# ZikangYuan/sr_livo

Hardware: AMD Instinct MI355X
Metric: sweeps/s (full ESIKF solve of a 64k-pt Livox sweep vs 1M-pt voxel map) (higher is better)
Workload: dtype f64; 1 GPU; HEADLINE: stream of 4 distinct 65536-keypoint livox sweeps (own poses and priors), 978481-pt voxel map (1000000 target), max_num_residuals=2147483647, r=1, K=20; one full ESIKF solve per sweep, every sweep crosses PCIe once (uploaded on the copy stream during the solve before it: resident in HBM when its solve starts); sweeps drawn with seeds 20251309 + 100 j, keeping those that take sweep 0's 2 E; parallelism=single GPU

## Files before the change

include/srlivo_hip_debug.h:

```cpp
#ifndef SRLIVO_HIP_DEBUG_H
#define SRLIVO_HIP_DEBUG_H

#include "srlivo_hip.h"

#ifdef __cplusplus
extern "C" {
#endif

int srl_debug_set_select_mode(srl_ctx *ctx, int select_mode);

int srl_debug_radix_sort_pairs(srl_ctx *ctx, const uint32_t *keys, int n, int bits, uint32_t *keys_sorted, uint32_t *positions_sorted);

int srl_debug_color_map_rebuilds(srl_ctx *ctx, int32_t *voxel_table, int32_t *grid_table);

int srl_debug_set_frame_order_mode(srl_ctx *ctx, int mode);
int srl_debug_frame_order_used(srl_ctx *ctx, int *used);

int srl_debug_set_gather_counts(srl_ctx *ctx, int nranks, int rank, const int64_t *counts);

int srl_debug_set_ablate(srl_ctx *ctx, int bits);
int srl_debug_set_fused_reduce(srl_ctx *ctx, int enable);
int srl_debug_set_bound_culling(srl_ctx *ctx, int enable);
int srl_debug_set_pose_box(srl_ctx *ctx, int kind);
int srl_debug_set_arm_linger(srl_ctx *ctx, double host_linger_us, double kernel_linger_us);
int srl_debug_pass_stamps(srl_ctx *ctx, int enable, long long *gpu_out, long long *host_out);
int srl_debug_frame_timing(srl_ctx *ctx, int enable, double out16[16]);
int srl_debug_set_frame_epoch(srl_ctx *ctx, int frames_to_wrap);
int srl_debug_set_launch_shape(srl_ctx *ctx, int keypoints_per_wave, int waves_per_workgroup);
int srl_debug_set_search_select_mode(srl_ctx *ctx, int select_mode);
int srl_debug_heap_topk(const double *distances, int n, int K, int32_t *out_index);
int srl_debug_device_sqrt(srl_ctx *ctx, const double *in, int n, double *out);
int srl_debug_block_times(srl_ctx *ctx, double *out, int max_blocks, int *nblocks);

#ifdef __cplusplus
}
#endif
#endif
```

sr_livo_amd/capi.py:

```python
import ctypes as C
import os
import re

import numpy as np

_HERE = os.path.dirname(os.path.abspath(__file__))
LIB_PATH = os.environ.get("SRL_LIB_PATH") or os.path.join(_HERE, "libsrlivo_hip.so")
INCLUDE_DIR = os.path.join(os.path.dirname(_HERE), "include")

SRL_OK = 0
SRL_ERR_NO_DEVICE = -1
SRL_ERR_UNSUPPORTED = -4
SRL_ERR_COMM = -7
SRL_ERR_NAN_PLANARITY = -8
SRL_ERR_NOT_ENOUGH_RESIDUALS = -9
SRL_COMM_ID_BYTES = 128


SRL_PEER_HANDLE_BYTES = 64


class SrlError(RuntimeError):
    def __init__(self, status, what, detail=""):
        self.status = status
# ... 112 lines not shown
        "srl_color_map_insert": ([p, p, C.c_int, C.c_double, C.c_double, p, p, C.c_int, p, C.c_int, C.POINTER(ColorTotals)], C.c_int),
        "srl_color_map_size": ([p, C.POINTER(C.c_int64), C.POINTER(C.c_int32), C.POINTER(C.c_int64), C.POINTER(C.c_int64)], C.c_int),
        "srl_color_map_download": ([p, p, p, p, C.c_int, p, p, C.c_int64], C.c_int),
        "srl_color_registered_download": ([p, C.c_int64, C.c_int, p], C.c_int),
        "srl_debug_color_map_rebuilds": ([p, C.POINTER(C.c_int32), C.POINTER(C.c_int32)], C.c_int),
        "srl_sweep_upload": ([p, p, C.c_int], C.c_int),
        "srl_sweep_shard": ([p, C.POINTER(C.c_int), C.POINTER(C.c_int), C.POINTER(C.c_int)], C.c_int),
        "srl_sweep_prefetch": ([p, p, C.c_int], C.c_int),
        "srl_sweep_swap": ([p], C.c_int),
        "srl_sweep_wait": ([p], C.c_int),
        "srl_thread_pin_to_gpu_numa": ([p, C.POINTER(C.c_int)], C.c_int),
        "srl_pinned_alloc": ([C.c_size_t, C.POINTER(p)], C.c_int),
        "srl_pinned_free": ([p], C.c_int),
        "srl_host_register": ([p, C.c_size_t], C.c_int),
        "srl_host_unregister": ([p], C.c_int),
        "srl_comm_backend_info": ([C.c_char_p, C.c_int, C.POINTER(C.c_int), C.POINTER(C.c_int)], C.c_int),
        "srl_build_residuals": ([p, C.POINTER(Frame), C.POINTER(IcpOpts), C.POINTER(NormalEq)], C.c_int),
        "srl_build_residuals_overlap": ([p, C.POINTER(Frame), C.POINTER(IcpOpts), C.POINTER(NormalEq), p, p], C.c_int),
        "srl_set_taps": ([p, C.c_int], C.c_int),
        "srl_fetch_neighbors": ([p, p, p, p], C.c_int),
        "srl_fetch_residuals": ([p, p, p, p, p, p, p], C.c_int),
        "srl_search_neighbors": ([p, p, C.c_int, C.c_int, C.c_double, C.c_int, C.c_int, p, p, p], C.c_int),
        "srl_transform_points": ([p, p, C.c_int, dp, dp, dp, dp, p], C.c_int),
        "srl_frame_upload": ([p, p, C.c_int], C.c_int),
        "srl_frame_undistort": ([p, p, p, p, C.c_int, p, C.c_int, C.c_double, C.c_int, dp, dp, p, p], C.c_int),
        "srl_frame_take": ([p, p, C.c_int], C.c_int),
        "srl_frame_subsample": ([p, p, C.c_int, C.c_double, C.POINTER(C.c_int)], C.c_int),
        "srl_frame_take_subsampled": ([p, p, C.c_int, p, p, p], C.c_int),
        "srl_frame_size": ([p, C.POINTER(C.c_int)], C.c_int),
        "srl_frame_select_keypoints": ([p, dp, dp, dp, dp, C.c_double, p, C.POINTER(C.c_int)], C.c_int),
        "srl_frame_commit_report": ([p, dp, dp, dp, dp, C.c_double, C.c_int, C.c_double, C.c_int, p, p, p, C.POINTER(C.c_int),
                                     C.POINTER(C.c_int)], C.c_int),
        "srl_frame_commit": ([p, dp, dp, dp, dp, C.c_double, C.c_int, C.c_double, C.c_int, p, C.POINTER(C.c_int)], C.c_int),
        "srl_comm_unique_id": ([p], C.c_int),
        "srl_comm_init_rank": ([p, C.c_int, C.c_int, p], C.c_int),
        "srl_comm_destroy": ([p], C.c_int),
        "srl_comm_set_library": ([C.c_char_p], C.c_int),
        "srl_comm_suspend": ([p, C.c_int], C.c_int),
        "srl_comm_info": ([p, C.POINTER(C.c_int), C.POINTER(C.c_int), C.POINTER(C.c_int), C.POINTER(C.c_int), C.POINTER(C.c_int64)], C.c_int),
        "srl_comm_set_host_callbacks": ([p, C.c_int, C.c_int, ALLREDUCE_FN, ALLGATHER_FN, p], C.c_int),
        "srl_debug_set_gather_counts": ([p, C.c_int, C.c_int, C.POINTER(C.c_int64)], C.c_int),
        "srl_peer_export": ([p, p, C.POINTER(p)], C.c_int),
        "srl_peer_attach": ([p, C.c_int, C.c_int, p, C.POINTER(p)], C.c_int),
        "srl_peer_set_deadline_ms": ([p, C.c_int], C.c_int),
        "srl_peer_stats": ([p, C.POINTER(C.c_int64), C.POINTER(C.c_int)], C.c_int),
        "srl_peer_detach": ([p], C.c_int),
        "srl_shard_range": ([C.c_int, C.c_int, C.c_int, C.POINTER(C.c_int), C.POINTER(C.c_int)], None),
        "srl_shard_budget": ([C.c_int, C.POINTER(C.c_int64), C.c_int, C.c_int, C.POINTER(C.c_int64), C.POINTER(C.c_int)], None),
        "srl_get_timing": ([p, C.POINTER(Timing)], C.c_int),
        "srl_debug_block_times": ([p, p, C.c_int, C.POINTER(C.c_int)], C.c_int),
        "srl_debug_set_ablate": ([p, C.c_int], C.c_int),
        "srl_debug_set_fused_reduce": ([p, C.c_int], C.c_int),
        "srl_debug_set_bound_culling": ([p, C.c_int], C.c_int),
        "srl_debug_set_pose_box": ([p, C.c_int], C.c_int),
        "srl_debug_set_arm_linger": ([p, C.c_double, C.c_double], C.c_int),
        "srl_debug_pass_stamps": ([p, C.c_int, p, p], C.c_int),
        "srl_debug_frame_timing": ([p, C.c_int, p], C.c_int),
        "srl_debug_set_frame_epoch": ([p, C.c_int], C.c_int),
        "srl_set_armed_launch": ([p, C.c_int], C.c_int),
        "srl_disarm": ([p], C.c_int),
        "srl_solve_end": ([p], C.c_int),
        "srl_get_arm_stats": ([p, C.POINTER(C.c_uint64)], C.c_int),
        "srl_debug_set_launch_shape": ([p, C.c_int, C.c_int], C.c_int),
        "srl_debug_set_search_select_mode": ([p, C.c_int], C.c_int),
        "srl_debug_set_select_mode": ([p, C.c_int], C.c_int),
        "srl_debug_set_frame_order_mode": ([p, C.c_int], C.c_int),
        "srl_debug_radix_sort_pairs": ([p, p, C.c_int, C.c_int, p, p], C.c_int),
        "srl_debug_frame_order_used": ([p, C.POINTER(C.c_int)], C.c_int),
        "srl_debug_heap_topk": ([p, C.c_int, C.c_int, p], C.c_int),
        "srl_debug_device_sqrt": ([p, p, C.c_int, p], C.c_int),
        "srl_set_profiling": ([p, C.c_int], C.c_int),
        "srl_set_profiling_period": ([p, C.c_int], C.c_int),
        "srl_timing_mark": ([p], C.c_int),
        "srl_lio_create": ([C.c_int, C.POINTER(p)], C.c_int),
        "srl_lio_destroy": ([p], C.c_int),
        "srl_lio_ctx": ([p], p),
        "srl_lio_last_error": ([p], C.c_char_p),
        "srl_lio_set_extrinsics": ([p, dp, dp], C.c_int),
        "srl_lio_set_laser_point_cov": ([p, C.c_double], C.c_int),
        "srl_lio_last_solve_launches": ([p, C.POINTER(C.c_int)], C.c_int),
        "srl_lio_eskf_get_state": ([p, dp], C.c_int),
        "srl_lio_eskf_set_state": ([p, dp], C.c_int),
        "srl_lio_eskf_get_cov": ([p, dp], C.c_int),
        "srl_lio_eskf_set_cov": ([p, dp], C.c_int),
        "srl_lio_eskf_set_noise": ([p, C.c_double, C.c_double, C.c_double, C.c_double], C.c_int),
        "srl_lio_eskf_init_imu": ([p, dp, dp], C.c_int),
        "srl_lio_eskf_scale_init_cov": ([p], C.c_int),
        "srl_lio_eskf_predict": ([p, C.c_double, dp, dp], C.c_int),
        "srl_lio_eskf_observe": ([p, dp], C.c_int),
        "srl_lio_add_points_to_map": ([p, p, C.c_int, C.c_double, C.c_int, C.c_double, C.c_int], C.c_int),
        "srl_lio_map_size": ([p, C.POINTER(C.c_int64)], C.c_int),
        "srl_lio_remove_points_far_from_location": ([p, dp, C.c_double], C.c_int),
        "srl_lio_set_collect_points_world": ([p, C.c_int], C.c_int),
        "srl_lio_points_world": ([p, p, C.c_int, C.POINTER(C.c_int)], C.c_int),
        "srl_lio_set_device_subsample": ([p, C.c_int], C.c_int),
        "srl_lio_set_color_map_options": ([p, C.POINTER(ColorOpts)], C.c_int),
        "srl_lio_set_color_times": ([p, C.c_double, C.c_double, C.c_int], C.c_int),
        "srl_lio_add_points_to_map_at": ([p, p, C.c_int, C.c_double, C.c_int, C.c_double, C.c_int, C.c_double, C.c_int], C.c_int),
        "srl_lio_color_visited": ([p, C.c_int, p, C.c_int, C.POINTER(C.c_int), C.POINTER(C.c_int)], C.c_int),
        "srl_lio_color_stored": ([p, p, C.c_int, C.POINTER(C.c_int)], C.c_int),
        "srl_lio_probe_checksum_of_committed_frame": ([p, C.c_int, C.c_double, C.POINTER(C.c_uint64), C.POINTER(C.c_int32)], C.c_int),
        "srl_lio_resident_sweep": ([p, p, C.c_int], C.c_int),
        "srl_lio_prefetch_sweep": ([p, p, C.c_int], C.c_int),
        "srl_lio_swap_sweep": ([p], C.c_int),
        "srl_lio_prefetch_sweep_during_solve": ([p, p, C.c_int], C.c_int),
        "srl_lio_update_iekf": ([p, C.POINTER(IcpOpts), p, C.c_int, dp, dp, C.c_int, p, C.c_int,
# ... 344 lines not shown
            self._chk(self.lib.srl_debug_set_select_mode(self.h, mode), "srl_debug_set_select_mode")
            self._select_mode = mode

    def build_residuals(self, frame, opts, allow=(SRL_ERR_NAN_PLANARITY,)):
        self._select(opts)
        out = NormalEq()
        rc = self._chk(self.lib.srl_build_residuals(self.h, C.byref(frame), C.byref(opts), C.byref(out)), "srl_build_residuals", ok=allow)
        return out, rc

    def build_residuals_overlap(self, frame, opts, fn, allow=(SRL_ERR_NAN_PLANARITY,)):
        self._select(opts)
        out = NormalEq()
        cb = C.CFUNCTYPE(None, C.c_void_p)(lambda _u: fn())
        rc = self._chk(self.lib.srl_build_residuals_overlap(self.h, C.byref(frame), C.byref(opts), C.byref(out), cb, None),
                       "srl_build_residuals_overlap", ok=allow)
        return out, rc

    def pin_thread_to_gpu_numa(self):
        node = C.c_int(-1)
        rc = self.lib.srl_thread_pin_to_gpu_numa(self.h, C.byref(node))
        return node.value if rc == 0 else None

    def fetch_neighbors(self, K=20):
        _, n, _ = self.sweep_shard()
        ids = np.empty((n, K), dtype=np.int32)
        status = np.empty(n, dtype=np.uint8)
        ncand = np.empty(n, dtype=np.int32)
        self._chk(self.lib.srl_fetch_neighbors(self.h, _ptr(ids), _ptr(status), _ptr(ncand)), "srl_fetch_neighbors")
        return ids, status, ncand

    def fetch_residuals(self):
        _, n, _ = self.sweep_shard()
        normal = np.empty((n, 3)); a2d = np.empty(n); w = np.empty(n); off = np.empty(n); d = np.empty(n); J = np.empty((n, 6))
        self._chk(self.lib.srl_fetch_residuals(self.h, _ptr(normal), _ptr(a2d), _ptr(w), _ptr(off), _ptr(d), _ptr(J)), "srl_fetch_residuals")
        return dict(normal=normal, a2D=a2d, weight=w, norm_offset=off, distance=d, jacobian=J)

    def search_neighbors(self, world_xyz, nb=1, size=1.0, K=20, thr=1):
        q = _f64(world_xyz, (-1, 3))
        ids = np.empty((len(q), K), dtype=np.int32)
        xyz = np.empty((len(q), K, 3), dtype=np.float32)
        nf = np.empty(len(q), dtype=np.int32)
        self._chk(self.lib.srl_search_neighbors(self.h, _ptr(q), len(q), nb, size, K, thr, _ptr(ids), _ptr(xyz), _ptr(nf)), "srl_search_neighbors")
        return ids, xyz, nf

    def set_launch_shape(self, kpw, wpb):
        self._chk(self.lib.srl_debug_set_launch_shape(self.h, int(kpw), int(wpb)), "srl_debug_set_launch_shape")

    def set_fused_reduce(self, on):
        self._chk(self.lib.srl_debug_set_fused_reduce(self.h, 1 if on else 0), "srl_debug_set_fused_reduce")

    def set_bound_culling(self, on):
        self._chk(self.lib.srl_debug_set_bound_culling(self.h, 1 if on else 0), "srl_debug_set_bound_culling")

    def set_search_select_mode(self, mode):
        self._chk(self.lib.srl_debug_set_search_select_mode(self.h, int(mode)), "srl_debug_set_search_select_mode")

    def set_armed_launch(self, on):
        mode = int(on) if on in (0, 1, 2) and not isinstance(on, bool) else (1 if on else 0)
        self._chk(self.lib.srl_set_armed_launch(self.h, mode), "srl_set_armed_launch")

    def solve_end(self):
        self._chk(self.lib.srl_solve_end(self.h), "srl_solve_end")

    def disarm(self):
        self._chk(self.lib.srl_disarm(self.h), "srl_disarm")

    def arm_stats(self):
        out = (C.c_uint64 * 4)()
        self._chk(self.lib.srl_get_arm_stats(self.h, out), "srl_get_arm_stats")
        return dict(zip(("armed", "fired", "cancelled", "expired"), (int(v) for v in out)))

    def set_pose_box(self, kind):
        self._chk(self.lib.srl_debug_set_pose_box(self.h, int(kind)), "srl_debug_set_pose_box")

    FRAME_STAGES = ("upload", "select_group", "select_download", "select_host_order", "select_gather", "commit_transform", "commit_download",
                    "insert_sort", "insert_segments", "insert_lookup_create", "insert_replay")

    def set_frame_epoch(self, frames_to_wrap):
        self._chk(self.lib.srl_debug_set_frame_epoch(self.h, int(frames_to_wrap)), "srl_debug_set_frame_epoch")

    def frame_timing(self, enable=True):
        out = np.zeros(16)
        self._chk(self.lib.srl_debug_frame_timing(self.h, 1 if enable else 0, _ptr(out)), "srl_debug_frame_timing")
        return dict(zip(self.FRAME_STAGES, (float(v) for v in out)))

    def pass_stamps(self, enable=True, read=True):
        g = np.zeros((64, 32), dtype=np.int64); h = np.zeros((64, 4), dtype=np.int64)
        self._chk(self.lib.srl_debug_pass_stamps(self.h, 1 if enable else 0, _ptr(g) if read else None, _ptr(h) if read else None), "srl_debug_pass_stamps")
        return g, h

    def set_arm_linger(self, host_linger_us=150.0, kernel_linger_us=300.0):
        self._chk(self.lib.srl_debug_set_arm_linger(self.h, float(host_linger_us), float(kernel_linger_us)), "srl_debug_set_arm_linger")

    def device_sqrt(self, x):
        x = _f64(x).ravel()
        out = np.empty_like(x)
        self._chk(self.lib.srl_debug_device_sqrt(self.h, _ptr(x), len(x), _ptr(out)), "srl_debug_device_sqrt")
        return out

    def transform_points(self, raw_xyz, q, t, R_il=None, t_il=None):
        r = _f64(raw_xyz, (-1, 3))
        out = np.empty_like(r)
        R_il = _f64(np.eye(3) if R_il is None else R_il).ravel()
        t_il = _f64(np.zeros(3) if t_il is None else t_il)
        self._chk(self.lib.srl_transform_points(self.h, _ptr(r), len(r), _dptr(_f64(q)), _dptr(_f64(t)), _dptr(R_il), _dptr(t_il), _ptr(out)), "srl_transform_points")
        return out
# ... 503 lines not shown
```

sr_livo_amd/csrc/srl_capi.cpp:

```cpp
#include "../../include/srlivo_hip.h"
#include "../../include/srlivo_hip_debug.h"
#include "host/srl_la.h"
#include "srl_device.h"
#include "srl_hash.h"
#include "srl_heap.h"

#include <hip/hip_runtime.h>
#include <sched.h>

#include <algorithm>
#include <atomic>
#include <chrono>
#include <climits>
#include <cstdio>
#include <cstdlib>
#include <cstring>
#include <mutex>
#include <string>
#include <vector>

struct SrlMapState;
int srl_map_insert_device(struct srl_ctx *ctx, const double *world_xyz, int n, double voxel_size, int cap,
                          double min_distance_points, int min_num_points, int *num_added);

// ... 835 lines not shown
    a.table = ctx->d_table;
    a.table_mask = ctx->table_cap - 1;
    a.slabs = ctx->d_slabs;
    a.inf_off = ctx->slab_cap * (unsigned)SRL_SLAB_BYTES;
    a.write_rec = ((ctx->taps || p.cut) && !p.fuse_cut) ? 1 : 0;
    {
        const srl::Quat q(f->q[0], f->q[1], f->q[2], f->q[3]);
        const srl::Mat3 Rn = q.normalized().toRotationMatrix();
        const srl::Mat3 R = q.toRotationMatrix();
        std::memcpy(a.Rn, Rn.a, sizeof a.Rn);
        std::memcpy(a.R, R.a, sizeof a.R);
    }
    std::memcpy(a.t, f->t, sizeof a.t);
    std::memcpy(a.t_last, f->t_last, sizeof a.t_last);
    std::memcpy(a.R_il, f->R_il, sizeof a.R_il);
    std::memcpy(a.t_il, f->t_il, sizeof a.t_il);
    a.size_voxel = o->size_voxel_map;
    a.max_dist = o->max_dist_to_plane_icp;
    {
        double lw = std::abs(o->weight_alpha), ln = std::abs(o->weight_neighborhood);
        const double sum = lw + ln;
        lw /= sum;
        ln /= sum;
        a.lambda_w = lw;
        a.lambda_n = ln;
    }
    a.power_planarity = o->power_planarity;
    a.nbr_scale = o->max_dist_to_plane_icp * o->min_number_neighbors;
    a.K = p.K;
    a.min_nb = o->min_number_neighbors;
    a.thr_cap = p.thr;
    a.select_mode = ctx->select_mode;
    a.ablate = ctx->ablate;
    a.stamps = ctx->h_arm_stamps;
    a.rec = ctx->d_rec;
    a.status = ctx->d_status;
    a.partials = ctx->d_partials;
    a.binfo = ctx->d_binfo;
    if (ctx->taps) {
        a.tap_ids = ctx->d_tap_ids;
        a.tap_ncand = ctx->d_tap_ncand;
        a.tap_normal = ctx->d_tap_normal;
        a.tap_a2d = ctx->d_tap_a2d;
        a.tap_offset = ctx->d_tap_offset;
    }
    {
        float sv = (float)o->size_voxel_map;
        int sv_bits; std::memcpy(&sv_bits, &sv, 4);
        const int sig[4] = {p.K, p.nb, p.thr, sv_bits};
        if (std::memcmp(sig, ctx->bound_sig, sizeof sig) != 0) { ctx->bound_n = 0; std::memcpy(ctx->bound_sig, sig, sizeof sig); }
        a.bound_out = ctx->d_bound;
        a.bound_in = ctx->bound_mode != 0 ? ctx->d_bound : nullptr;
        a.bound_use = a.bound_in ? std::min(ctx->bound_n, n_eff) : 0;
    }
    if (p.fused) {
        a.granules = ctx->d_granules;
        a.mailbox = p.transport == Transport::rccl ? ctx->d_mail : ctx->h_mail;
        a.mail_tagged = p.tagged_mail ? 1 : 0;
    }
    if (p.fuse_cut) {
        a.rec_granules = ctx->d_rec_granules;
        a.cut_max = o->max_num_residuals;
    }
}

static int grow_pass_buffers(srl_ctx *ctx, const PassPlan &p) {
    int rc;
    ctx->taps_valid = false;
    if (ctx->taps) {
        if ((rc = ensure_taps(ctx, ctx->n, p.K))) return rc;
        if (ctx->n > 0) {
            HIPCHK(ctx, hipMemsetAsync(ctx->d_tap_ids, 0xFF, (size_t)ctx->n * p.K * sizeof(int), ctx->stream));
            HIPCHK(ctx, hipMemsetAsync(ctx->d_tap_normal, 0, (size_t)ctx->n * 3 * sizeof(double), ctx->stream));
            HIPCHK(ctx, hipMemsetAsync(ctx->d_tap_a2d, 0, (size_t)ctx->n * sizeof(double), ctx->stream));
            HIPCHK(ctx, hipMemsetAsync(ctx->d_tap_offset, 0, (size_t)ctx->n * sizeof(double), ctx->stream));
        }
    }
    ctx->last_nblocks = p.nblocks;
    if (p.nblocks > ctx->block_cap) {
        if ((rc = ensure(ctx, ctx->d_partials, (size_t)p.nblocks * SRL_PART_STRIDE))) return rc;
        if ((rc = ensure(ctx, ctx->d_binfo, (size_t)p.nblocks))) return rc;
        ctx->block_cap = p.nblocks;
    }
    if (ctx->profiling == 2 && ctx->ring_head - ctx->ring_tail >= (unsigned)srl_ctx::PROF_RING && (rc = drain_ring(ctx, true))) return rc;
    if (p.fused && p.transport == Transport::rccl && !ctx->d_mail && (rc = ensure(ctx, ctx->d_mail, 1))) return rc;
    const size_t need = (size_t)p.nblocks * p.kpb * 16;
    if (p.fuse_cut && need > ctx->rec_granule_cap) {
        if ((rc = ensure(ctx, ctx->d_rec_granules, need))) return rc;
        HIPCHK(ctx, hipMemsetAsync(ctx->d_rec_granules, 0, need * sizeof(unsigned long long), ctx->stream));
        ctx->rec_granule_cap = need;
    }
    return SRL_OK;
}

struct ExchangeTag { unsigned long long seq; unsigned epoch; int slot; };
static ExchangeTag exchange_tag(unsigned long long seq) {
    if ((unsigned)seq == 0u) ++seq;
    return {seq, (unsigned)seq, (int)(seq & 1ull)};
}
static ExchangeTag next_exchange(srl_ctx *ctx) {
    const ExchangeTag t = exchange_tag(ctx->peer_seq + 1);
    ctx->peer_seq = t.seq;
    return t;
}

static SrlAssocArgs arm_signature(const SrlAssocArgs &src) {
// ... 436 lines not shown
    a.size_voxel = size_voxel_map; a.K = K; a.thr_cap = threshold_voxel_capacity; a.select_mode = ctx->search_select_mode;
    a.ids = d_ids; a.nb_xyz = d_xyz; a.num_found = d_nf;
    HIPCHK(ctx, srl_launch_search(a, nb_voxels_visited, ctx->stream));
    HIPCHK(ctx, hipMemcpyAsync(ids, d_ids, (size_t)n * K * sizeof(int), hipMemcpyDeviceToHost, ctx->stream));
    HIPCHK(ctx, hipMemcpyAsync(num_found, d_nf, (size_t)n * sizeof(int), hipMemcpyDeviceToHost, ctx->stream));
    if (nb_xyz) HIPCHK(ctx, hipMemcpyAsync(nb_xyz, d_xyz, (size_t)n * K * 3 * sizeof(float), hipMemcpyDeviceToHost, ctx->stream));
    HIPCHK(ctx, hipStreamSynchronize(ctx->stream));
    return SRL_OK;
}

int srl_transform_points(srl_ctx *ctx, const double *raw_xyz, int n, const double q[4], const double t[3],
                         const double R_il[9], const double t_il[3], double *out_xyz) {
    if (!ctx || n < 0 || (n > 0 && (!raw_xyz || !out_xyz)) || !q || !t || !R_il || !t_il) return SRL_ERR_BAD_ARG;
    SRL_DISARM(ctx);
    if (n == 0) return SRL_OK;
    HIPCHK(ctx, hipSetDevice(ctx->device));
    DevBuf b_in, b_o;
    HIPCHK(ctx, b_in.alloc(ctx, (size_t)n * 3 * sizeof(double)));
    HIPCHK(ctx, b_o.alloc(ctx, (size_t)n * 3 * sizeof(double)));
    double *d_in = b_in.as<double>(), *d_o = b_o.as<double>();
    HIPCHK(ctx, hipMemcpyAsync(d_in, raw_xyz, (size_t)n * 3 * sizeof(double), hipMemcpyHostToDevice, ctx->stream));
    SrlXform X;
    const srl::Mat3 R = srl::Quat(q[0], q[1], q[2], q[3]).toRotationMatrix();
    std::memcpy(X.R, R.a, sizeof X.R);
    std::memcpy(X.t, t, sizeof X.t);
    std::memcpy(X.R_il, R_il, sizeof X.R_il);
    std::memcpy(X.t_il, t_il, sizeof X.t_il);
    HIPCHK(ctx, srl_launch_transform(d_in, n, X, d_o, ctx->stream));
    HIPCHK(ctx, hipMemcpyAsync(out_xyz, d_o, (size_t)n * 3 * sizeof(double), hipMemcpyDeviceToHost, ctx->stream));
    HIPCHK(ctx, hipStreamSynchronize(ctx->stream));
    return SRL_OK;
}

int srl_debug_set_ablate(srl_ctx *ctx, int bits) {
    if (!ctx) return SRL_ERR_BAD_ARG;
    SRL_DISARM(ctx);
    ctx->ablate = bits;
    return SRL_OK;
}
int srl_debug_set_launch_shape(srl_ctx *ctx, int keypoints_per_wave, int waves_per_workgroup) {
    if (!ctx) return SRL_ERR_BAD_ARG;
    SRL_DISARM(ctx);
    if (keypoints_per_wave != 0 && keypoints_per_wave != 2 && keypoints_per_wave != 3 && keypoints_per_wave != 6 && keypoints_per_wave != 12 && keypoints_per_wave != 4 && keypoints_per_wave != 8 && keypoints_per_wave != 16) return SRL_ERR_BAD_ARG;
    if (waves_per_workgroup != 0 && waves_per_workgroup != 4 && waves_per_workgroup != 16) return SRL_ERR_BAD_ARG;
    ctx->force_kpw = keypoints_per_wave;
    ctx->force_wpb = waves_per_workgroup;
    return SRL_OK;
}
int srl_debug_set_bound_culling(srl_ctx *ctx, int enable) {
    if (!ctx) return SRL_ERR_BAD_ARG;
    SRL_DISARM(ctx);
    ctx->bound_mode = enable ? 1 : 0;
    ctx->bound_n = 0;
    return SRL_OK;
}
int srl_debug_set_fused_reduce(srl_ctx *ctx, int enable) {
    if (!ctx) return SRL_ERR_BAD_ARG;
    SRL_DISARM(ctx);
    ctx->fuse_reduce = enable != 0;
    return SRL_OK;
}
int srl_debug_set_select_mode(srl_ctx *ctx, int select_mode) {
    if (!ctx || select_mode < 0 || select_mode > 5) return SRL_ERR_BAD_ARG;
    SRL_DISARM(ctx);
    ctx->select_mode = select_mode;
    return SRL_OK;
}
int srl_debug_set_frame_order_mode(srl_ctx *ctx, int mode) {
    if (!ctx || mode < 0 || mode > 1) return SRL_ERR_BAD_ARG;
    ctx->frame_order_mode = mode;
    return SRL_OK;
}
int srl_debug_frame_order_used(srl_ctx *ctx, int *used) {
    if (!ctx || !used) return SRL_ERR_BAD_ARG;
    *used = ctx->frame_order_used;
    return SRL_OK;
}
int srl_debug_set_search_select_mode(srl_ctx *ctx, int select_mode) {
    if (!ctx || select_mode < 0 || select_mode > 5) return SRL_ERR_BAD_ARG;
    ctx->search_select_mode = select_mode;
    return SRL_OK;
}
int srl_debug_heap_topk(const double *distances, int n, int K, int32_t *out_index) {
    if (n < 0 || K < 1 || K > SRL_MAX_NEIGHBORS || (n > 0 && !distances) || !out_index) return SRL_ERR_BAD_ARG;
    double hd[SRL_MAX_NEIGHBORS];
    int he[SRL_MAX_NEIGHBORS];
    int size = 0;
    for (int i = 0; i < n; i++) size = srl_heap_offer(hd, he, size, K, distances[i], i);
    int out[SRL_MAX_NEIGHBORS];
    srl_heap_drain(hd, he, size, out);
    for (int i = 0; i < size; i++) out_index[i] = out[i];
    return size;
}
int srl_debug_device_sqrt(srl_ctx *ctx, const double *in, int n, double *out) {
    if (!ctx || n < 0 || (n > 0 && (!in || !out))) return SRL_ERR_BAD_ARG;
    SRL_DISARM(ctx);
    if (n == 0) return SRL_OK;
    HIPCHK(ctx, hipSetDevice(ctx->device));
    DevBuf b;
    HIPCHK(ctx, b.alloc(ctx, (size_t)n * sizeof(double)));
    HIPCHK(ctx, hipMemcpyAsync(b.as<double>(), in, (size_t)n * sizeof(double), hipMemcpyHostToDevice, ctx->stream));
    HIPCHK(ctx, srl_launch_sqrt(b.as<double>(), n, ctx->stream));
    HIPCHK(ctx, hipMemcpyAsync(out, b.as<double>(), (size_t)n * sizeof(double), hipMemcpyDeviceToHost, ctx->stream));
    HIPCHK(ctx, hipStreamSynchronize(ctx->stream));
    return SRL_OK;
}
// ... 361 lines not shown
```

sr_livo_amd/csrc/srl_ctx.h:

```cpp
#pragma once
#include "../../include/srlivo_hip.h"
#include "srl_device.h"
#include "host/tr1_relation.h"

#include <hip/hip_runtime.h>
#include "srl_rccl.h"

#include <string>
#include <vector>

struct SrlEpochTable {
    unsigned long long *keyw = nullptr;
    unsigned long long *minw = nullptr;
    unsigned cap = 0;
    unsigned epoch16 = 0;
    unsigned counter32 = 0;
};

#define SRL_PEER_POISON_WORD SRL_PEER_INBOX_GRANULES
#define SRL_PEER_DEVICE_WORD (SRL_PEER_INBOX_GRANULES + 1)
#define SRL_PEER_INBOX_ALLOC_GRANULES (SRL_PEER_INBOX_GRANULES + 8)

struct srl_ctx {
    int device = 0;
    bool counted = false;
    hipStream_t stream = nullptr;
    std::string err;

    SrlMapSlot *d_table = nullptr;
    unsigned table_cap = 0;
    unsigned char *d_slabs = nullptr;
    unsigned slab_cap = 0;
    int num_voxels = 0;
    long long num_points = 0;

    double *d_raw = nullptr;
    int sweep_cap = 0;
    int n = 0;
    int shard_begin = 0;
    int total_n = 0;
    bool sweep_loaded = false;
    int search_select_mode = 0;
    int select_mode = 0;
    int ablate = 0;
    void (*overlap_fn)(void *) = nullptr;
    void *overlap_user = nullptr;

    double *d_raw_next = nullptr;
    double *d_stage_next = nullptr;
    double *d_stage_cur = nullptr;
    int soa_valid_n = 0;
    int next_cap = 0, stage_next_cap = 0, stage_cur_cap = 0;
    int next_n = -1, next_begin = 0, next_total = 0;
    hipStream_t copy_stream = nullptr;
    hipStream_t prefix_stream = nullptr;
    int num_cu = 256;
    hipEvent_t next_ready = nullptr;
    hipEvent_t up_ev[2][2] = {};
    bool up_one_dma[2] = {true, true};
    int next_slot = 0;
    int next_prefix_n = 0;
    int prefix_hint = 0;
    float *d_bound = nullptr;
    int bound_n = 0;
    int bound_sig[4] = {0, 0, 0, 0};
    int bound_mode = 1;
    bool tail_pending = false;
    int cur_slot = 0, cur_prefix_n = 0;

    double *d_frame_raw = nullptr;
    double *d_frame_world = nullptr;
    int frame_cap = 0;
    int frame_n = -1;
    int frame_world_n = -1;
    bool frame_world_seen = false;
    struct SrlColorMap *color = nullptr;
    double *d_corr_in = nullptr, *d_corr_rel = nullptr, *d_corr_imu = nullptr, *d_corr_raw = nullptr;
    int *d_corr_seg = nullptr;
    int corr_cap = 0;
    int corr_n = -1;
    int *d_sub_kept = nullptr;
    unsigned *d_sub_seen = nullptr;
    int sub_cap = 0;
    int sub_n = -1;
    unsigned sub_seen_tag = 0;

    bool frame_timing = false;
    double frame_stage_us[16] = {};
    long long frame_stage_last_ns = 0;

    hipEvent_t upload_ev = nullptr;
    bool upload_pending = false;

    static constexpr int RING_SLOTS = 4;
    static constexpr int RING_SLOT_BYTES = 256 * 1024;
    char *h_ring = nullptr;
    hipEvent_t ring_ev[RING_SLOTS] = {};
    bool ring_busy[RING_SLOTS] = {};
    unsigned ring_next = 0;

    char *h_scratch = nullptr;
    size_t h_scratch_bytes = 0;
    char *h_frame_x = nullptr;
    size_t h_frame_x_bytes = 0;
    unsigned *d_frame_sync = nullptr;
    unsigned frame_tag = 0;
    SrlTr1Sched *d_tr1_sched = nullptr;
    int tr1_steps = -1;
    unsigned tr1_first[SRL_TR1_MAX_STEPS] = {0}, tr1_nb[SRL_TR1_MAX_STEPS + 1] = {0};
    int frame_order_mode = 0;
    int frame_order_used = 0;
    int *h_insert_cnt = nullptr;
    hipEvent_t ev_insert = nullptr, ev_world = nullptr;
    bool insert_pending = false;
    hipEvent_t ev_frame_read = nullptr;
    SrlEpochTable sel_table, ins_table;

    double *d_rec = nullptr;
    unsigned char *d_status = nullptr;
// ... 225 lines not shown
```

sr_livo_amd/csrc/srl_device.h:

```cpp
#pragma once
#include <hip/hip_runtime.h>
#include <stddef.h>
#include <stdint.h>


#define SRL_CAP 20
#define SRL_SLAB_BYTES 256
#define SRL_MAX_SLABS 16777215u
#ifndef SRL_KPB
#define SRL_KPB 64
#endif
#ifndef SRL_ASSOC_WAVES_PER_SIMD
#define SRL_ASSOC_WAVES_PER_SIMD 4
#endif
#define SRL_BLOCK 256
#define SRL_SURV_CAP 64
#define SRL_WAVE_SCRATCH 2048
#define SRL_MAXK 32
#define SRL_EMPTY_KEY 0xFFFFFFFFFFFFFFFFull
#define SRL_TABLE_FACTOR 4u
#define SRL_PART_STRIDE 32
#define SRL_ROW_GRANULES 128
#define SRL_FUSED_MAX_BLOCKS 2048
#define SRL_FUSED_GROUP 256
// ... 70 lines not shown
#define SRL_PEER_TIMEOUT_MARK 0x9EE9ll
struct SrlPeerTable {
    unsigned long long *inbox[SRL_MAX_PEERS];
    int nranks, rank;
};

struct SrlAssocArgs {
    const double *raw_x, *raw_y, *raw_z;
    const double *aos;
    int n;
    const SrlMapSlot *table;
    unsigned table_mask;
    const unsigned char *slabs;
    int write_rec;
    unsigned inf_off;
    double Rn[9];
    double R[9];
    double t[3];
    double t_last[3];
    double R_il[9];
    double t_il[3];
    double size_voxel;
    double max_dist;
    double lambda_w, lambda_n;
    double power_planarity;
    double nbr_scale;
    int K;
    int min_nb;
    int thr_cap;
    int select_mode;
    int ablate;
    unsigned long long *granules;
    unsigned long long *rec_granules;
    long long cut_max;
    SrlMailbox *mailbox;
    int mail_tagged;
    int pad_mail;
    unsigned long long seq;
    const unsigned long long *pose_box;
    const double *alt_x, *alt_y, *alt_z;
    const double *alt_aos;
    unsigned long long *pose_relay;
    int pose_relayed;
    int pad_relay;
    unsigned pose_epoch;
    unsigned arm_linger_ticks;
    long long *stamps;
    const SrlPeerTable *peer;
    unsigned peer_epoch;
    int peer_slot;
    const float *bound_in;
    float *bound_out;
    int bound_use;
    int pad_bound;
    double *rec;
    unsigned char *status;
    double *partials;
    SrlBlockInfo *binfo;
    int *tap_ids;
    int *tap_ncand;
    double *tap_normal;
    double *tap_a2d;
    double *tap_offset;
};

#define SRL_POSE_DOUBLES 24
static_assert(sizeof(SrlAssocArgs) <= 4096, "the struct travels in the kernarg segment");

struct SrlReduceArgs {
    const double *rec;
    const unsigned char *status;
    const double *partials;
    const SrlBlockInfo *binfo;
    int n;
    int nblocks;
    long long max_res;
    const long long *gather;
    int rank;
    int max_num_residuals;
    SrlDevOut *out;
    SrlMailbox *mailbox;
    unsigned long long seq;
    int kpb;
};

struct SrlSearchArgs {
    const double *q;
    int n;
    const SrlMapSlot *table;
    unsigned table_mask;
    const unsigned char *slabs;
    double size_voxel;
    int K;
    int thr_cap;
    int select_mode;
    int *ids;
    float *nb_xyz;
    int *num_found;
};

hipError_t srl_launch_assoc(const SrlAssocArgs &a, int nb_voxels, int kpw, int wpb, hipStream_t s);
int srl_assoc_lds_bytes(int K, int nb_voxels, int kpw, int wpb);
static inline int srl_keypoints_per_wave(int n) { return n <= 16384 ? 4 : (n <= 32768 ? 8 : 16); }
static inline int srl_keypoints_per_wave_one_round(int n, int num_cu) {
    const int set[7] = {2, 3, 4, 6, 8, 12, 16};
    for (int i = 0; i < 7; ++i) if ((long long)16 * set[i] * num_cu >= n) return set[i];
    return 16;
// ... 14 lines not shown
```

sr_livo_amd/csrc/srl_kernels.hip:

```cpp
#include "srl_device.h"
#include "srl_hash.h"
#include "srl_heap.h"

#include <math.h>
#include <type_traits>

namespace {

struct alignas(8) VoxEnt { unsigned slab; unsigned count; };
struct Surv { double d2; float x, y, z; unsigned id; };
static_assert(sizeof(Surv) == 24, "survivor record is 24 bytes");
static_assert(SRL_SURV_CAP * 24 + (SRL_MAXK + 1) * 8 <= SRL_WAVE_SCRATCH, "general-path scratch (survivors + sorted d2) must fit");
static_assert(64 * 8 + SRL_MAXK * 16 + SRL_MAXK * 4 <= SRL_WAVE_SCRATCH, "heap replay scratch must fit");

__device__ __forceinline__ int lane_id() {
    return __builtin_amdgcn_mbcnt_hi(~0u, __builtin_amdgcn_mbcnt_lo(~0u, 0));
}
__device__ __forceinline__ int lanes_below(unsigned long long m) {
    return __builtin_amdgcn_mbcnt_hi((unsigned)(m >> 32), __builtin_amdgcn_mbcnt_lo((unsigned)m, 0));
}

struct Cand { bool valid; double d2; float x, y, z; unsigned id; };

__device__ __forceinline__ Cand eval_cand(int e, int nv, const VoxEnt *vox, const unsigned char *slabs,
// ... 223 lines not shown
                if (od < bd2 || (od == bd2 && oe < be)) { bd2 = od; be = oe; }
            }
            if (r > 0 && !(bd2 > last_d2 * SRL_NEAR_TIE)) { tie = true; break; }
            if (r < nsel && (be & 63) == lane) {
                const Cand c = eval_cand(be, nv, vox, slabs, qx, qy, qz);
                sink.put(r, c.x, c.y, c.z, c.id);
            }
            last_d2 = bd2;
            last_e = be;
        }
        fallback_out = 1;
    }
    __builtin_amdgcn_wave_barrier();
    if (tie) {
        select_topk_replay(qx, qy, qz, nv, vox, slabs, K, surv, lane, sink, total_out);
        fallback_out = 1;
    }
}

struct LaneRole {
    int pdx, pdy, pdz;
    int c0, slot;
};
__device__ __forceinline__ LaneRole lane_role(int lane) {
    LaneRole r;
    const int pl = lane & 31;
    const int ix = pl / 9, iy = (pl / 3) % 3, iz = pl % 3;
    r.pdx = ix - 1; r.pdy = iy - 1; r.pdz = iz - 1;
    r.c0 = lane / SRL_CAP;
    r.slot = lane - r.c0 * SRL_CAP;
    return r;
}

struct ProbeReq {
    unsigned long long key;
    unsigned h;
    SrlMapSlot s0, s1;
};
__device__ __forceinline__ ProbeReq probe_issue(const int *kv, int kl, const LaneRole &role, const SrlMapSlot *table,
                                                unsigned mask, int lane) {
    ProbeReq r;
    r.key = SRL_EMPTY_KEY; r.h = 0;
    r.s0.key = SRL_EMPTY_KEY; r.s0.slab = 0; r.s0.count = 0;
    r.s1 = r.s0;
    if ((lane & 31) < 27) {
        const int *k = kv + (kl + (lane >> 5)) * 4;
        r.key = srl_pack_key((short)(k[0] + role.pdx), (short)(k[1] + role.pdy), (short)(k[2] + role.pdz));
        r.h = srl_hash_key(r.key) & mask;
        r.s0 = table[r.h];
        r.s1 = table[(r.h + 1) & mask];
    }
    return r;
}
__device__ __forceinline__ int probe_finish(const ProbeReq &r, int thr_cap, const SrlMapSlot *table, unsigned mask,
                                            VoxEnt *vox, int lane, int *ncand_pair, bool cull = false, const float *qf_pair = nullptr,
                                            const int *kv_pair = nullptr, const LaneRole *role = nullptr, float size_voxel = 1.0f) {
    const bool prober = (lane & 31) < 27;
    const bool m0 = prober && r.s0.key == r.key;
    const bool m1 = prober && !m0 && r.s0.key != SRL_EMPTY_KEY && r.s1.key == r.key;
    bool found = m0 || m1;
    unsigned slab = m0 ? r.s0.slab : r.s1.slab, cnt = m0 ? r.s0.count : r.s1.count;
    const bool more = prober && !found && r.s0.key != SRL_EMPTY_KEY && r.s1.key != SRL_EMPTY_KEY;
    if (__ballot(more) != 0ull) {
        if (more) {
            unsigned h = (r.h + 2) & mask;
            for (unsigned probe = 2; probe <= mask; ++probe) {
                const SrlMapSlot sl = table[h];
                if (sl.key == r.key) { slab = sl.slab; cnt = sl.count; found = true; break; }
                if (sl.key == SRL_EMPTY_KEY) break;
                h = (h + 1) & mask;
            }
        }
    }
    found = found && (int)cnt >= thr_cap && cnt > 0;
    {
#if defined(__HIP_DEVICE_COMPILE__)
        int v = found ? (int)cnt : 0;
        v += __builtin_amdgcn_update_dpp(0, v, 0x111, 0xF, 0xF, false);
        v += __builtin_amdgcn_update_dpp(0, v, 0x112, 0xF, 0xF, false);
        v += __builtin_amdgcn_update_dpp(0, v, 0x114, 0xF, 0xF, false);
        v += __builtin_amdgcn_update_dpp(0, v, 0x118, 0xF, 0xF, false);
        v += __builtin_amdgcn_update_dpp(0, v, 0x142, 0xA, 0xF, false);
        if ((lane & 31) == 31) ncand_pair[lane >> 5] = v;
#endif
    }
    if (cull) {
        const int hh = lane >> 5;
        const float *qf = qf_pair + 8 * hh;
        const int *kv = kv_pair + 4 * hh;
        const float r2 = qf[5];
        float bd2 = 0.0f;
        const int pd[3] = {role->pdx, role->pdy, role->pdz};
#pragma unroll
        for (int ax = 0; ax < 3; ++ax) {
            const int v = kv[ax] + pd[ax];
            const float lo = (float)(v > 0 ? v : v - 1) * size_voxel, hi = (float)(v < 0 ? v : v + 1) * size_voxel;
            const float d = fmaxf(fmaxf(lo - qf[ax], qf[ax] - hi), 0.0f);
            bd2 += d * d;
        }
        found = found && bd2 <= r2;
    }
    const unsigned long long m = __ballot(found);
    const unsigned m_lo = (unsigned)m, m_hi = (unsigned)(m >> 32);
    const int nv_a = __popc(m_lo), nv_b = __popc(m_hi);
    if (prober) {
        const bool upper = lane >= 32;
        const unsigned f_lo = found ? m_lo : (~m_lo & 0x7FFFFFFu), f_hi = found ? m_hi : (~m_hi & 0x7FFFFFFu);
        const int below = upper ? (int)__builtin_amdgcn_mbcnt_hi(f_hi, 0u) : (int)__builtin_amdgcn_mbcnt_lo(f_lo, 0u);
        const int nv_own = upper ? nv_b : nv_a;
        VoxEnt ve; ve.slab = found ? slab : 0u; ve.count = found ? cnt : 0u;
        vox[(upper ? 32 : 0) + (found ? below : nv_own + below)] = ve;
    }
    __builtin_amdgcn_wave_barrier();
    return nv_a | (nv_b << 8);
}

struct LdsSink {
    float *col;
    int row;
    int plane;
    int *tap_ids;
    __device__ __forceinline__ void put(int rank, float x, float y, float z, unsigned id) {
        float *p = col + rank * row;
        p[0] = x;
        p[plane] = y;
        p[2 * plane] = z;
        if (tap_ids) tap_ids[rank] = (int)id;
    }
};

struct alignas(16) SurvRec { float x, y, z; int code; };
#define SRL_PAIR_MAX_ROUNDS 4

__device__ __forceinline__ float d2_f32(float px, float py, float pz, float qx, float qy, float qz) {
#pragma clang fp contract(fast)
    const float dx = px - qx, dy = py - qy, dz = pz - qz;
    return dx * dx + dy * dy + dz * dz;
}

template <class Sink>
__device__ __forceinline__ int finish_survivors(double qx, double qy, double qz, int c, const VoxEnt *vox, int K, void *scratch,
                                                int lane, Sink &sink, double *tau_out = nullptr) {
    SurvRec *recs = reinterpret_cast<SurvRec *>(__builtin_assume_aligned(scratch, 16));
// ... 690 lines not shown
                const float bq[3] = {bp.x, bp.y, bp.z};
                bool inside = true;
#pragma unroll
                for (int ax = 0; ax < 3; ++ax) {
                    const int vlo = kv[ax] - NB, vhi = kv[ax] + NB;
                    const float lo = (float)(vlo > 0 ? vlo : vlo - 1) * sz, hi = (float)(vhi < 0 ? vhi : vhi + 1) * sz;
                    inside = inside && (bq[ax] - rt) - slack >= lo && (bq[ax] + rt) + slack <= hi;
                }
                if (inside) {
                    const float r = rt + sqrtf(ex * ex + ey * ey + ez * ez) * 1.000001f + slack;
                    r2 = (r * r) * 1.00001f;
                }
            }
            qf[5] = r2;
            *reinterpret_cast<double *>(qf + 6) = __builtin_huge_val();
        }
        s_kv[kq * 4 + 0] = kv[0];
        s_kv[kq * 4 + 1] = kv[1];
        s_kv[kq * 4 + 2] = kv[2];
        s_nfound[kq] = 0;
        s_ncand[kq] = 0;
    } else if (wave == WPB - 1 && lane < KPW + 2) {
        const int kq = KPB + (lane - KPW);
        s_kv[kq * 4 + 0] = 0; s_kv[kq * 4 + 1] = 0; s_kv[kq * 4 + 2] = 0;
    }
    __syncthreads();
    tile_stamp(11);

    {
        const int left = n_pass() - bbase_kp;
        const int n_here = __builtin_amdgcn_readfirstlane(left < KPB ? left : KPB);
        auto make_sink = [&](int kl) {
            LdsSink sink;
            sink.col = s_nb + kl;
            sink.row = NB_ROW;
            sink.plane = nb_plane;
            sink.tap_ids = A.tap_ids ? (A.tap_ids + (size_t)(bbase_kp + kl) * Kn) : nullptr;
            return sink;
        };
        auto keypoint_general = [&](int kl, bool tie) {
            const double qx = s_pw[kl * 3 + 0], qy = s_pw[kl * 3 + 1], qz = s_pw[kl * 3 + 2];
            LdsSink sink = make_sink(kl);
            int total = 0, fb = 0;
            const int nv = probe_voxels<NB>(qx, qy, qz, A.size_voxel, A.thr_cap, A.table, A.table_mask, vox, lane);
            select_topk(qx, qy, qz, nv, vox, A.slabs, Kn, tie ? 5 : A.select_mode, surv, lane, sink, total, fb);
            n_fallback += (NB == 1) ? 1 : fb;
            if (lane == 0) {
                s_nfound[kl] = total < Kn ? total : Kn;
                s_ncand[kl] = total;
            }
        };
        if constexpr (NB == 1 && FAST != 0) {
            const LaneRole role = lane_role(lane);
            const int npairs = n_here > 0 ? (n_here + 1) >> 1 : 0;
            auto take = [&]() { int p = 0; if (lane == 0) p = atomicAdd(s_next, 1); return __builtin_amdgcn_readfirstlane(p); };
            int cur = take();
            ProbeReq preq;
            if (!(abl & 32)) preq = probe_issue(s_kv, 2 * (cur < npairs ? cur : npairs), role, A.table, A.table_mask, lane);
            while (cur < npairs) {
                const int nxt = take();
                const int nv_pair = __builtin_amdgcn_readfirstlane((abl & 8) ? 0 : probe_finish(preq, A.thr_cap, A.table, A.table_mask, vox, lane, s_ncand + 2 * cur, use_bounds, s_qf + 16 * cur,
                                                                                                               s_kv + 8 * cur, &role, (float)A.size_voxel));
                if (!(abl & 32)) preq = probe_issue(s_kv, 2 * (nxt < npairs ? nxt : npairs), role, A.table, A.table_mask, lane);
                auto file = [&](int kl, int done, int total) {
                    (void)total;
                    if (done == SEL_DONE) {
                    } else {
                        s_defer[atomicAdd(s_next + 1, 1)] = (unsigned short)(kl | (done == SEL_TIE ? 0x8000 : 0));
                    }
                };
                const int r_a = (int)((((unsigned)nv_pair & 0xFFu) + 2u) * 0x5556u >> 16), r_b = (int)(((((unsigned)nv_pair >> 8) & 0xFFu) + 2u) * 0x5556u >> 16);
                const int r_max = r_a > r_b ? r_a : r_b;
                if (2 * cur + 1 < n_here && r_max <= SRL_PAIR_MAX_ROUNDS && !(abl & (4 | 256))) {
                    const int kl = 2 * cur;
                    LdsSink sink_a = make_sink(kl), sink_b = make_sink(kl + 1);
                    int total_a = 0, total_b = 0, done;
                    if (r_max <= 2) done = select_pair_f32_r<2>(s_pw + kl * 3, s_pw + kl * 3 + 3, s_qf + kl * 8, s_qf + kl * 8 + 8, vox, A.slabs, A.inf_off, Kn, surv, lane, role, sink_a, sink_b, total_a, total_b, abl);
                    else if (r_max <= 3) done = select_pair_f32_r<3>(s_pw + kl * 3, s_pw + kl * 3 + 3, s_qf + kl * 8, s_qf + kl * 8 + 8, vox, A.slabs, A.inf_off, Kn, surv, lane, role, sink_a, sink_b, total_a, total_b, abl);
                    else done = select_pair_f32_r<4>(s_pw + kl * 3, s_pw + kl * 3 + 3, s_qf + kl * 8, s_qf + kl * 8 + 8, vox, A.slabs, A.inf_off, Kn, surv, lane, role, sink_a, sink_b, total_a, total_b, abl);
                    (void)total_a; (void)total_b;
                    if (done != (SEL_DONE | (SEL_DONE << 8))) {
                        if (lane == 0) {
                            if ((done & 0xFF) != SEL_DONE) s_defer[atomicAdd(s_next + 1, 1)] = (unsigned short)(kl | ((done & 0xFF) == SEL_TIE ? 0x8000 : 0));
                            if ((done >> 8) != SEL_DONE) s_defer[atomicAdd(s_next + 1, 1)] = (unsigned short)((kl + 1) | ((done >> 8) == SEL_TIE ? 0x8000 : 0));
                        }
                    }
                } else {
#pragma nounroll
                    for (int h = 0; h < 2; ++h) {
                        const int kl = 2 * cur + h;
                        if (kl >= n_here) break;
                        const int nv_fast = h ? (nv_pair >> 8) : (nv_pair & 0xFF);
                        const double qx = s_pw[kl * 3 + 0], qy = s_pw[kl * 3 + 1], qz = s_pw[kl * 3 + 2];
                        LdsSink sink = make_sink(kl);
                        int total = nv_fast;
                        int done = SEL_DONE;
                        if (!(abl & 4)) done = select_topk_f32(qx, qy, qz, s_qf + kl * 8, nv_fast, vox + 32 * h, A.slabs, A.inf_off, Kn, surv, lane, role, sink, total, abl);
                        if (lane == 0) file(kl, done, total);
                    }
                }
                cur = nxt;
            }
        } else if constexpr (NB == 2 && FAST != 0) {
            const LaneRole role = lane_role(lane);
            auto take = [&]() { int p = 0; if (lane == 0) p = atomicAdd(s_next, 1); return __builtin_amdgcn_readfirstlane(p); };
            for (int kl = take(); kl < n_here; kl = take()) {
                const double qx = s_pw[kl * 3 + 0], qy = s_pw[kl * 3 + 1], qz = s_pw[kl * 3 + 2];
                int total_all = 0;
                const int nv = probe_voxels<NB>(qx, qy, qz, A.size_voxel, A.thr_cap, A.table, A.table_mask, vox, lane, use_bounds ? s_qf + kl * 8 : nullptr, &total_all);
                if (lane < 3) { VoxEnt z; z.slab = 0u; z.count = 0u; vox[nv + lane] = z; }
                __builtin_amdgcn_wave_barrier();
                LdsSink sink = make_sink(kl);
                int total = 0;
                const int done = select_topk_f32_loop(qx, qy, qz, s_qf + kl * 8, nv, vox, A.slabs, A.inf_off, Kn, surv, lane, role, sink, total);
                total = total_all;
                if (lane == 0) {
// ... 1187 lines not shown
```

Baseline: 10730 sweeps/s.

## Derive first-pass culling bound from home voxel's K points when no prior bound

When a keypoint has no carried-over search radius (qf[5] is infinite) and its home voxel already holds at least K points, the probe loads those points, takes the max squared distance across the half-wave with DPP reductions, and uses it as a conservative culling radius for neighbor voxels. This lets the first ESIKF pass prune candidate voxels that were previously all kept. The next probe issue is also moved inside probe_finish, after the home-slab loads, to overlap memory latency. The cost is extra slab loads and reductions per pair. Debug hooks to toggle the feature and fetch the bounds are added.

```diff
diff --git a/include/srlivo_hip_debug.h b/include/srlivo_hip_debug.h
--- a/include/srlivo_hip_debug.h
+++ b/include/srlivo_hip_debug.h
@@ -21,6 +21,8 @@
 int srl_debug_set_ablate(srl_ctx *ctx, int bits);
 int srl_debug_set_fused_reduce(srl_ctx *ctx, int enable);
 int srl_debug_set_bound_culling(srl_ctx *ctx, int enable);
+int srl_debug_set_first_pass_bound(srl_ctx *ctx, int enable);
+int srl_debug_fetch_bounds(srl_ctx *ctx, float *out, int max_entries, int *n_valid);
 int srl_debug_set_pose_box(srl_ctx *ctx, int kind);
 int srl_debug_set_arm_linger(srl_ctx *ctx, double host_linger_us, double kernel_linger_us);
 int srl_debug_pass_stamps(srl_ctx *ctx, int enable, long long *gpu_out, long long *host_out);
diff --git a/sr_livo_amd/capi.py b/sr_livo_amd/capi.py
--- a/sr_livo_amd/capi.py
+++ b/sr_livo_amd/capi.py
@@ -188,6 +188,8 @@
         "srl_debug_set_ablate": ([p, C.c_int], C.c_int),
         "srl_debug_set_fused_reduce": ([p, C.c_int], C.c_int),
         "srl_debug_set_bound_culling": ([p, C.c_int], C.c_int),
+        "srl_debug_set_first_pass_bound": ([p, C.c_int], C.c_int),
+        "srl_debug_fetch_bounds": ([p, C.c_void_p, C.c_int, C.POINTER(C.c_int)], C.c_int),
         "srl_debug_set_pose_box": ([p, C.c_int], C.c_int),
         "srl_debug_set_arm_linger": ([p, C.c_double, C.c_double], C.c_int),
         "srl_debug_pass_stamps": ([p, C.c_int, p, p], C.c_int),
@@ -638,6 +640,16 @@
     def set_bound_culling(self, on):
         self._chk(self.lib.srl_debug_set_bound_culling(self.h, 1 if on else 0), "srl_debug_set_bound_culling")
 
+    def set_first_pass_bound(self, on):
+        self._chk(self.lib.srl_debug_set_first_pass_bound(self.h, 1 if on else 0), "srl_debug_set_first_pass_bound")
+
+    def fetch_bounds(self):
+        _, n, _ = self.sweep_shard()
+        out = np.empty((max(n, 1), 4), dtype=np.float32)
+        m = C.c_int(0)
+        self._chk(self.lib.srl_debug_fetch_bounds(self.h, _ptr(out), n, C.byref(m)), "srl_debug_fetch_bounds")
+        return out[: m.value].copy()
+
     def set_search_select_mode(self, mode):
         self._chk(self.lib.srl_debug_set_search_select_mode(self.h, int(mode)), "srl_debug_set_search_select_mode")
 
diff --git a/sr_livo_amd/csrc/srl_capi.cpp b/sr_livo_amd/csrc/srl_capi.cpp
--- a/sr_livo_amd/csrc/srl_capi.cpp
+++ b/sr_livo_amd/csrc/srl_capi.cpp
@@ -911,6 +911,7 @@
         a.bound_out = ctx->d_bound;
         a.bound_in = ctx->bound_mode != 0 ? ctx->d_bound : nullptr;
         a.bound_use = a.bound_in ? std::min(ctx->bound_n, n_eff) : 0;
+        a.home_bound = ctx->home_bound_mode != 0 ? 1 : 0;
     }
     if (p.fused) {
         a.granules = ctx->d_granules;
@@ -1453,6 +1454,24 @@
     SRL_DISARM(ctx);
     ctx->bound_mode = enable ? 1 : 0;
     ctx->bound_n = 0;
+    return SRL_OK;
+}
+int srl_debug_set_first_pass_bound(srl_ctx *ctx, int enable) {
+    if (!ctx) return SRL_ERR_BAD_ARG;
+    SRL_DISARM(ctx);
+    ctx->home_bound_mode = enable ? 1 : 0;
+    return SRL_OK;
+}
+int srl_debug_fetch_bounds(srl_ctx *ctx, float *out, int max_entries, int *n_valid) {
+    if (!ctx || !n_valid || max_entries < 0 || (max_entries > 0 && !out)) return SRL_ERR_BAD_ARG;
+    SRL_DISARM(ctx);
+    HIPCHK(ctx, hipSetDevice(ctx->device));
+    const int n = ctx->d_bound ? std::min(ctx->bound_n, max_entries) : 0;
+    *n_valid = n;
+    if (n > 0) {
+        HIPCHK(ctx, hipMemcpyAsync(out, ctx->d_bound, (size_t)n * 4 * sizeof(float), hipMemcpyDeviceToHost, ctx->stream));
+        HIPCHK(ctx, hipStreamSynchronize(ctx->stream));
+    }
     return SRL_OK;
 }
 int srl_debug_set_fused_reduce(srl_ctx *ctx, int enable) {
diff --git a/sr_livo_amd/csrc/srl_ctx.h b/sr_livo_amd/csrc/srl_ctx.h
--- a/sr_livo_amd/csrc/srl_ctx.h
+++ b/sr_livo_amd/csrc/srl_ctx.h
@@ -65,6 +65,7 @@
     int bound_n = 0;
     int bound_sig[4] = {0, 0, 0, 0};
     int bound_mode = 1;
+    int home_bound_mode = 1;
     bool tail_pending = false;
     int cur_slot = 0, cur_prefix_n = 0;
 
diff --git a/sr_livo_amd/csrc/srl_device.h b/sr_livo_amd/csrc/srl_device.h
--- a/sr_livo_amd/csrc/srl_device.h
+++ b/sr_livo_amd/csrc/srl_device.h
@@ -146,7 +146,7 @@
     const float *bound_in;
     float *bound_out;
     int bound_use;
-    int pad_bound;
+    int home_bound;
     double *rec;
     unsigned char *status;
     double *partials;
diff --git a/sr_livo_amd/csrc/srl_kernels.hip b/sr_livo_amd/csrc/srl_kernels.hip
--- a/sr_livo_amd/csrc/srl_kernels.hip
+++ b/sr_livo_amd/csrc/srl_kernels.hip
@@ -299,9 +299,12 @@
     }
     return r;
 }
+__device__ __forceinline__ float d2_f32(float px, float py, float pz, float qx, float qy, float qz);
+template <class Mid>
 __device__ __forceinline__ int probe_finish(const ProbeReq &r, int thr_cap, const SrlMapSlot *table, unsigned mask,
-                                            VoxEnt *vox, int lane, int *ncand_pair, bool cull = false, const float *qf_pair = nullptr,
-                                            const int *kv_pair = nullptr, const LaneRole *role = nullptr, float size_voxel = 1.0f) {
+                                            VoxEnt *vox, int lane, int *ncand_pair, bool cull, const float *qf_pair,
+                                            const int *kv_pair, const LaneRole *role, float size_voxel, int home_K,
+                                            const unsigned char *slabs, Mid &&mid) {
     const bool prober = (lane & 31) < 27;
     const bool m0 = prober && r.s0.key == r.key;
     const bool m1 = prober && !m0 && r.s0.key != SRL_EMPTY_KEY && r.s1.key == r.key;
@@ -320,6 +323,24 @@
         }
     }
     found = found && (int)cnt >= thr_cap && cnt > 0;
+    float hx = 0.0f, hy = 0.0f, hz = 0.0f;
+    bool home_want = false, home_ld = false;
+    if (home_K > 0) {
+#if defined(__HIP_DEVICE_COMPILE__)
+        const unsigned hcnt = found ? cnt : 0u;
+        const unsigned hc_a = (unsigned)__builtin_amdgcn_readlane((int)hcnt, 13), hc_b = (unsigned)__builtin_amdgcn_readlane((int)hcnt, 45);
+        const unsigned hs_a = (unsigned)__builtin_amdgcn_readlane((int)slab, 13), hs_b = (unsigned)__builtin_amdgcn_readlane((int)slab, 45);
+        const bool upper = lane >= 32;
+        const unsigned hc = upper ? hc_b : hc_a, hs = upper ? hs_b : hs_a;
+        home_want = (int)hc >= home_K && qf_pair[8 * (lane >> 5) + 5] == __builtin_huge_valf();
+        home_ld = home_want && (unsigned)(lane & 31) < (hc < (unsigned)SRL_CAP ? hc : (unsigned)SRL_CAP);
+        if (home_ld) {
+            const float *p = reinterpret_cast<const float *>(slabs + (hs * (unsigned)SRL_SLAB_BYTES + (unsigned)(lane & 31) * 12u));
+            hx = p[0]; hy = p[1]; hz = p[2];
+        }
+#endif
+    }
+    mid();
     {
 #if defined(__HIP_DEVICE_COMPILE__)
         int v = found ? (int)cnt : 0;
@@ -335,7 +356,23 @@
         const int hh = lane >> 5;
         const float *qf = qf_pair + 8 * hh;
         const int *kv = kv_pair + 4 * hh;
-        const float r2 = qf[5];
+        float r2 = qf[5];
+#if defined(__HIP_DEVICE_COMPILE__)
+        if (__ballot(home_want) != 0ull) {
+            float d = home_ld ? d2_f32(hx, hy, hz, qf[0], qf[1], qf[2]) : 0.0f;
+            d = fmaxf(d, __int_as_float(__builtin_amdgcn_update_dpp(0, __float_as_int(d), 0x111, 0xF, 0xF, false)));
+            d = fmaxf(d, __int_as_float(__builtin_amdgcn_update_dpp(0, __float_as_int(d), 0x112, 0xF, 0xF, false)));
+            d = fmaxf(d, __int_as_float(__builtin_amdgcn_update_dpp(0, __float_as_int(d), 0x114, 0xF, 0xF, false)));
+            d = fmaxf(d, __int_as_float(__builtin_amdgcn_update_dpp(0, __float_as_int(d), 0x118, 0xF, 0xF, false)));
+            d = fmaxf(d, __int_as_float(__builtin_amdgcn_update_dpp(0, __float_as_int(d), 0x142, 0xA, 0xF, false)));
+            const float t_a = __int_as_float(__builtin_amdgcn_readlane(__float_as_int(d), 31)), t_b = __int_as_float(__builtin_amdgcn_readlane(__float_as_int(d), 63));
+            if (home_want) {
+                const float slack = 1e-3f + 1e-6f * (fabsf(qf[0]) + fabsf(qf[1]) + fabsf(qf[2]));
+                const float rr = sqrtf(qf[3] + qf[4] * (hh ? t_b : t_a)) * 1.000001f + slack;
+                r2 = (rr * rr) * 1.00001f;
+            }
+        }
+#endif
         float bd2 = 0.0f;
         const int pd[3] = {role->pdx, role->pdy, role->pdz};
 #pragma unroll
@@ -1132,6 +1169,7 @@
         };
         if constexpr (NB == 1 && FAST != 0) {
             const LaneRole role = lane_role(lane);
+            const int home_K = A.home_bound != 0 ? Kn : 0;
             const int npairs = n_here > 0 ? (n_here + 1) >> 1 : 0;
             auto take = [&]() { int p = 0; if (lane == 0) p = atomicAdd(s_next, 1); return __builtin_amdgcn_readfirstlane(p); };
             int cur = take();
@@ -1139,9 +1177,12 @@
             if (!(abl & 32)) preq = probe_issue(s_kv, 2 * (cur < npairs ? cur : npairs), role, A.table, A.table_mask, lane);
             while (cur < npairs) {
                 const int nxt = take();
-                const int nv_pair = __builtin_amdgcn_readfirstlane((abl & 8) ? 0 : probe_finish(preq, A.thr_cap, A.table, A.table_mask, vox, lane, s_ncand + 2 * cur, use_bounds, s_qf + 16 * cur,
-                                                                                                               s_kv + 8 * cur, &role, (float)A.size_voxel));
-                if (!(abl & 32)) preq = probe_issue(s_kv, 2 * (nxt < npairs ? nxt : npairs), role, A.table, A.table_mask, lane);
+                auto issue_next = [&]() { if (!(abl & 32)) preq = probe_issue(s_kv, 2 * (nxt < npairs ? nxt : npairs), role, A.table, A.table_mask, lane); };
+                int nv_pair = 0;
+                if (abl & 8) issue_next();
+                else nv_pair = probe_finish(preq, A.thr_cap, A.table, A.table_mask, vox, lane, s_ncand + 2 * cur, use_bounds || home_K > 0, s_qf + 16 * cur,
+                                            s_kv + 8 * cur, &role, (float)A.size_voxel, home_K, A.slabs, issue_next);
+                nv_pair = __builtin_amdgcn_readfirstlane(nv_pair);
                 auto file = [&](int kl, int done, int total) {
                     (void)total;
                     if (done == SEL_DONE) {
```

Result: slower. 10390 sweeps/s (-3.2%).
